# hailanyi/CPD

Hardware: AMD Instinct MI355X
Metric: frames/sec voxelize->sparse3D->BEV->NMS, 160k-pt Waymo cloud (higher is better)
Workload: dtype f32 (split-fp16 x2 on the fp16 MFMA pipe: 3 products, fp32 accumulate)

## Files before the change

### cpd_amd/_lib.py

```python
import ctypes
import os

import torch

_HERE = os.path.dirname(os.path.abspath(__file__))
LIB_PATH = os.environ.get("CPD_HIP_LIB", os.path.join(_HERE, "csrc", "libcpd_hip.so"))

CPD_ERRORS = {-1: "CPD_ERR_ARG", -2: "CPD_ERR_WORKSPACE", -3: "CPD_ERR_LAUNCH", -4: "CPD_ERR_UNSUPPORTED"}


class CpdHipError(RuntimeError):
    pass


_lib = None

_VP, _I, _F, _SZ = ctypes.c_void_p, ctypes.c_int, ctypes.c_float, ctypes.c_size_t
_D = ctypes.c_double
_I3 = ctypes.POINTER(ctypes.c_int32)
_FP = ctypes.POINTER(ctypes.c_float)

SIGNATURES = {
    "cpd_launch_log_enable": (None, [_I]),
    "cpd_launch_log_note": (None, [ctypes.c_char_p]),
# ... 34 lines not shown
    "cpd_conv3x3_rows_scaled": (_I, [_VP, _I, _I, _I, _I, _I, _VP, _I, _VP, _VP, _VP, _I, _I, _VP, _I, _I, _VP, _VP]),
    "cpd_conv3x3_rows_ranged": (_I, [_VP, _I, _I, _I, _I, _I, _VP, _I, _VP, _VP, _VP, _I, _I, _VP, _I, _I, _VP, _VP, _VP]),
    "cpd_gather_conv_ranged": (_I, [_VP, _I, _I, _I, _VP, _VP, _VP, _I, _I, _I, _VP, _VP, _VP, _I, _I, _VP, _I, _VP, _I, _I, _VP, _VP, _VP]),
    "cpd_gather_conv_ws": (_I, [_VP, _I, _I, _I, _VP, _VP, _VP, _I, _I, _I, _VP, _VP, _VP, _I, _I, _VP, _I, _VP, _I, _I, _VP, _VP, _VP, _SZ, _VP]),
    "cpd_gather_conv_split_bytes": (_SZ, [_I, _I, _I, _I, _I, _I]),
    "cpd_absmax_rows": (_I, [_VP, _I, ctypes.c_longlong, _I, _VP, _VP]),
    "cpd_densify_nchw": (_I, [_VP, _VP, _I, _I, _I, _I3, _VP, _VP]),
    "cpd_densify_nhwc": (_I, [_VP, _VP, _I, _I, _I, _I3, _VP, _VP]),
    "cpd_densify_nhwc_cd": (_I, [_VP, _VP, _I, _I, _I, _I3, _VP, _VP]),
    "cpd_densify_nhwc_rows": (_I, [_VP, _VP, _I, _I, _I, _I3, _VP, _VP]),
    "cpd_densify_nhwc_clear": (_I, [_VP, _I, _I, _I, _I3, _VP, _VP]),
    "cpd_rulebook_conv2d": (_I, [_I, _I, _I, _I, _I, _I, _I, _VP, _VP]),
    "cpd_center_decode_workspace_bytes": (_SZ, [_I, _I, _I, _I]),
    "cpd_center_decode": (_I, [_VP, _VP, _VP, _VP, _VP, _I, ctypes.c_longlong, _I, _I, _I, _I, _I, _I, _F, _FP, _FP, _FP, _F,
                               _VP, _VP, _VP, _VP, _VP, _SZ, _VP]),
    "cpd_boxes_overlap_bev": (_I, [_VP, _I, _VP, _I, _VP, _VP]),
    "cpd_boxes_iou_bev": (_I, [_VP, _I, _VP, _I, _VP, _VP]),
    "cpd_boxes_iou3d": (_I, [_VP, _I, _VP, _I, _VP, _VP]),
    "cpd_nms_workspace_bytes": (_SZ, [_I]),
    "cpd_nms_rotated": (_I, [_VP, _I, _F, _VP, _VP, _VP, _SZ, _VP]),
    "cpd_nms_normal": (_I, [_VP, _I, _F, _VP, _VP, _VP, _SZ, _VP]),
    "cpd_nms_batch": (_I, [_VP, _VP, _I, _I, _F, _I, _VP, _VP, _VP, _SZ, _VP]),
    "cpd_nms_batch_first": (_I, [_VP, _VP, _I, _I, _F, _I, _I, _I, _VP, _VP, _VP, _VP, _SZ, _VP]),
    "cpd_nms_batch_where": (_I, [_VP, _VP, _VP, _I, _I, _F, _I, _VP, _VP, _VP, _SZ, _VP]),
    "cpd_rank_scores": (_I, [_VP, _I, _VP, _VP, _I, _I, _F, _I, _I, _VP, _VP, _VP, _VP, _VP]),
    "cpd_select_boxes": (_I, [_VP, _VP, _VP, _VP, _VP, _I, _I, _I, _I, _VP, _VP, _VP, _VP, _VP]),
    "cpd_boxes_iou_bev_cpu": (_I, [_VP, _I, _VP, _I, _VP]),
    "cpd_col_reduce_workspace_bytes": (_SZ, [_I, _I]),
    "cpd_col_sum": (_I, [_VP, _I, _I, _I, _VP, _VP, _SZ, _VP]),
    "cpd_bn_stats": (_I, [_VP, _I, _I, _I, _VP, _VP, _VP, _SZ, _VP]),
# ... 126 lines not shown
```

### cpd_amd/csrc/decode.hip

```cpp
#include "common.h"

namespace {

struct MapView {
    const float *p;
    int pix, ch;
    __device__ __forceinline__ MapView sample(int b, long long sample_stride) const {
        return MapView{p + (size_t)b * sample_stride, pix, ch};
    }
    __device__ __forceinline__ float at(int pixel, int channel) const {
        return p[(size_t)pixel * pix + (size_t)channel * ch];
    }
};

__device__ __forceinline__ uint32_t f2key(float f) {
    uint32_t u = __float_as_uint(f);
    return (u & 0x80000000u) ? ~u : (u | 0x80000000u);
}
__device__ __forceinline__ float key2f(uint32_t k) {
    uint32_t u = (k & 0x80000000u) ? (k & 0x7fffffffu) : ~k;
    return __uint_as_float(u);
}
__device__ __forceinline__ float sigmoidf(float x) { return 1.0f / (1.0f + expf(-x)); }

// ... 144 lines not shown
__global__ void __launch_bounds__(1024) topk_class_kernel(MapView hm_all, long long sample_stride, int num_class, int hw,
                                                          int K, float *__restrict__ s1, int32_t *__restrict__ i1) {
    __shared__ TopkSmem sm;
    __shared__ TopkHist hist;
    const int cls = blockIdx.x, b = blockIdx.y;
    const MapView hm = hm_all.sample(b, sample_stride);
    if (!block_topk_logits(hm, cls, hw, K, hist, sm)) block_topk(hw, K, SigKey{hm, cls}, sm);
    const size_t o = ((size_t)b * num_class + cls) * K;
    for (int k = threadIdx.x; k < K; k += blockDim.x) {
        unsigned long long p = sm.packed[k];
        s1[o + k] = key2f((uint32_t)(p >> 32));
        i1[o + k] = (int32_t)(~(uint32_t)p);
    }
}

struct DecodeParams {
    MapView center, center_z, dim, rot;
    long long sample_stride;
    int num_class, h, w, K;
    float stride, vx, vy, lox, loy;
    float lim[6];
    float score_thresh;
};

__global__ void __launch_bounds__(1024) decode_kernel(DecodeParams q, const float *__restrict__ s1,
                                                      const int32_t *__restrict__ i1, float *__restrict__ boxes,
                                                      float *__restrict__ scores, int32_t *__restrict__ labels,
                                                      int32_t *__restrict__ n_out) {
    __shared__ TopkSmem sm;
    const int K = q.K;
    const int bsmp = blockIdx.x;
    s1 += (size_t)bsmp * q.num_class * K;
    i1 += (size_t)bsmp * q.num_class * K;
    boxes += (size_t)bsmp * K * 7;
    scores += (size_t)bsmp * K;
    labels += (size_t)bsmp * K;
    n_out += bsmp;
    q.center = q.center.sample(bsmp, q.sample_stride);
    q.center_z = q.center_z.sample(bsmp, q.sample_stride);
    q.dim = q.dim.sample(bsmp, q.sample_stride);
    q.rot = q.rot.sample(bsmp, q.sample_stride);
    {
        const int n = q.num_class * K;
        for (int i2 = threadIdx.x; i2 < n; i2 += blockDim.x) {
            const int c = i2 / K, j = i2 - c * K;
            const uint32_t key = f2key(s1[i2]);
            int rank = j;
            for (int c2 = 0; c2 < q.num_class; ++c2) {
                if (c2 == c) continue;
                const float *l = s1 + (size_t)c2 * K;
                int lo = 0, hi = K;
                while (lo < hi) {
                    const int mid = (lo + hi) >> 1;
                    const uint32_t km = f2key(l[mid]);
                    if (c2 < c ? km >= key : km > key) lo = mid + 1; else hi = mid;
                }
                rank += lo;
            }
            if (rank < K) sm.packed[rank] = ((unsigned long long)key << 32) | (uint32_t)(~(uint32_t)i2);
        }
        __syncthreads();
    }
    const int k = threadIdx.x;
    float bx[7];
    float sc = 0.f;
    int cls = 0;
    uint32_t keep = 0;
    if (k < K) {
        unsigned long long p = sm.packed[k];
        sc = key2f((uint32_t)(p >> 32));
        const int i2 = (int)(~(uint32_t)p);
        cls = i2 / K;
        const int ind = i1[i2];
        const float xs = (float)(ind % q.w), ys = (float)(ind / q.w);
        bx[0] = (xs + q.center.at(ind, 0)) * q.stride * q.vx + q.lox;
        bx[1] = (ys + q.center.at(ind, 1)) * q.stride * q.vy + q.loy;
        bx[2] = q.center_z.at(ind, 0);
        bx[3] = expf(q.dim.at(ind, 0));
        bx[4] = expf(q.dim.at(ind, 1));
        bx[5] = expf(q.dim.at(ind, 2));
        bx[6] = atan2f(q.rot.at(ind, 1), q.rot.at(ind, 0));
        bool ok = bx[0] >= q.lim[0] && bx[1] >= q.lim[1] && bx[2] >= q.lim[2] && bx[0] <= q.lim[3] &&
                  bx[1] <= q.lim[4] && bx[2] <= q.lim[5];
        ok = ok && (sc > q.score_thresh);
        keep = ok ? 1u : 0u;
    }
    __syncthreads();
    uint32_t tot;
    uint32_t pos = block_excl_scan(keep, sm.scan, &tot);
    if (keep) {
#pragma unroll
        for (int c = 0; c < 7; ++c) boxes[(size_t)pos * 7 + c] = bx[c];
        scores[pos] = sc;
        labels[pos] = cls;
    }
    if (threadIdx.x == 0) *n_out = (int32_t)tot;
}

}

extern "C" size_t cpd_center_decode_workspace_bytes(int batch, int num_class, int hw, int k) {
    if (batch <= 0 || num_class <= 0 || hw <= 0 || k <= 0) return 0;
    return cpd_align((size_t)batch * num_class * k * 4) * 2;
}

extern "C" int cpd_center_decode(const float *hm, const float *center, const float *center_z, const float *dim,
                                 const float *rot, int batch, long long sample_stride, int pix_stride, int ch_stride,
                                 int num_class, int h, int w, int k,
                                 float feature_map_stride, const float voxel_xy[2], const float range_lo_xy[2],
                                 const float limit_range[6], float score_thresh, float *boxes, float *scores,
                                 int32_t *labels, int32_t *n_out, void *workspace, size_t workspace_bytes,
                                 cpd_stream_t stream) {
    if (!hm || !center || !center_z || !dim || !rot || !boxes || !scores || !labels || !n_out || !workspace ||
// ... 2 lines not shown
    const long long hw = (long long)h * w;
    if (k > 1024 || k > hw || (long long)num_class * k > (1 << 24) || hw >= (1ll << 31)) return CPD_ERR_UNSUPPORTED;
    if (workspace_bytes < cpd_center_decode_workspace_bytes(batch, num_class, (int)hw, k)) return CPD_ERR_WORKSPACE;
    hipStream_t s = cpd_s(stream);
    float *s1 = (float *)workspace;
    int32_t *i1 = (int32_t *)((char *)workspace + cpd_align((size_t)batch * num_class * k * 4));
    topk_class_kernel<<<dim3(num_class, batch), 1024, 0, s>>>(MapView{hm, pix_stride, ch_stride}, sample_stride, num_class,
                                                              (int)hw, k, s1, i1);
    DecodeParams q;
    q.center = MapView{center, pix_stride, ch_stride};
    q.center_z = MapView{center_z, pix_stride, ch_stride};
    q.dim = MapView{dim, pix_stride, ch_stride};
    q.rot = MapView{rot, pix_stride, ch_stride};
    q.sample_stride = sample_stride;
    q.num_class = num_class; q.h = h; q.w = w; q.K = k;
    q.stride = feature_map_stride; q.vx = voxel_xy[0]; q.vy = voxel_xy[1];
    q.lox = range_lo_xy[0]; q.loy = range_lo_xy[1];
    for (int i = 0; i < 6; ++i) q.lim[i] = limit_range[i];
    q.score_thresh = score_thresh;
    decode_kernel<<<batch, 1024, 0, s>>>(q, s1, i1, boxes, scores, labels, n_out);
    return cpd_check_launch();
}
```

### cpd_amd/engine.py

```python
import contextlib
import math
from dataclasses import dataclass, field
from typing import Dict, List

import torch

from . import _lib, ops


@dataclass
class ModelConfig:
    point_cloud_range: List[float] = field(default_factory=lambda: [-75.2, -75.2, -2.0, 75.2, 75.2, 4.0])
    voxel_size: List[float] = field(default_factory=lambda: [0.1, 0.1, 0.15])
    max_points_per_voxel: int = 5
    max_voxels: int = 1000000
    num_point_features: int = 5
    num_filters: List[int] = field(default_factory=lambda: [16, 32, 64, 128])
    out_features: int = 128
    bev_layer_nums: List[int] = field(default_factory=lambda: [5, 5])
    bev_layer_strides: List[int] = field(default_factory=lambda: [1, 2])
    bev_num_filters: List[int] = field(default_factory=lambda: [128, 256])
    bev_upsample_strides: List[int] = field(default_factory=lambda: [1, 2])
    bev_num_upsample_filters: List[int] = field(default_factory=lambda: [256, 256])
    shared_conv_channel: int = 64
# ... 17 lines not shown
    voxelizer_group: int = 64
    batched_voxelizer_min_frames: int = 2
    row_order: str = "taps"
    row_order_brick: tuple = (8, 8)
    row_order_level0: bool = False
    chunked_rulebooks: bool = True
    plan_channels: tuple = (32, 64)
    plan_tile_rows: int = 256
    plan_rulebooks: bool = False
    row_order_chunk: int = 4096
    row_order_min_rows: int = 65536
    index_side_stream: bool = True
    deblock_side_stream: bool = True
    deblock_side_stream_max_frames: int = 8
    index_side_stream_max_frames: int = 1 << 30

    @property
    def grid_zyx(self):
        return ops.voxel_grid_size(self.voxel_size, self.point_cloud_range)

    @property
    def sparse_shape(self):
        g = self.grid_zyx
        return [g[0] + 1, g[1], g[2]]

    def head_names(self):
        return list(self.head_order) + ["hm"]

    def head_out(self, name):
        return self.num_class if name == "hm" else self.head_channels[name]
# ... 90 lines not shown
    if conv_bias is not None:
        shift = shift + conv_bias.double() * scale
    return scale.float(), shift.float()


class _Layer:
    __slots__ = ("w", "kv", "c_in", "c_out", "scale", "shift", "relu")

    def __init__(self, w_kio, scale, shift, relu, device):
        w_kio = w_kio.to(device=device, dtype=torch.float32).contiguous()
        self.kv, self.c_in, self.c_out = w_kio.shape
        self.w = ops.pack_weight(w_kio)
        self.scale = scale.to(device).contiguous() if scale is not None else None
        self.shift = shift.to(device).contiguous() if shift is not None else None
        self.relu = relu


class CenterPointEngine:

    SPARSE_BN_EPS = 1e-3
    BEV_BN_EPS = 1e-3
    HEAD_BN_EPS = 1e-5

    def __init__(self, cfg: ModelConfig, state_dict: Dict[str, torch.Tensor], device="cuda", host_results=False):
        self.cfg = cfg
        self.device = torch.device(device)
        self.host_results = bool(host_results)
        self.sd = state_dict
        self.voxelizer = ops.Voxelizer(cfg.voxel_size, cfg.point_cloud_range, cfg.num_point_features,
                                       cfg.max_points_per_voxel, cfg.max_voxels, device=self.device)
# ... 73 lines not shown
        for hi, name in enumerate(names):
            q = p + "heads_list.0.%s." % name
            w = sd[q + "0.0.weight"]
            w1.append(w.permute(2, 3, 1, 0).reshape(9, sc, sc))
            s, t = _fold_bn(sd, q + "0.1", self.HEAD_BN_EPS, sd.get(q + "0.0.bias"))
            s1.append(s); t1.append(t)
            wo = sd[q + "1.weight"]
            co = wo.shape[0]
            w2[:, hi * sc:(hi + 1) * sc, col:col + co] = wo.permute(2, 3, 1, 0).reshape(9, sc, co)
            b2[col:col + co] = sd[q + "1.bias"]
            self.head_slices[name] = (col, co)
            col += co
        self.head1 = _Layer(torch.cat(w1, dim=2), torch.cat(s1), torch.cat(t1), True, dev)
        self.head2 = _Layer(w2, None, b2, False, dev)
        self.head_ld = 16 * ((n_out + 15) // 16)

    def _final_shape(self):
        shape = self.cfg.sparse_shape
        for stage in ["conv2", "conv3", "conv4", "conv_out"]:
            k, s, pd = _DOWN[stage]
            shape = ops.conv_out_shape(shape, k, s, pd)
        return shape

    def _final_depth(self):
        return self._final_shape()[0]

    def _side_stream(self):
        return _lib.side_stream(self.device, "index")

    def _range_reset(self):
        self._rb = None
        self._rb_next = 0
        if self.cfg.conv_math == "f16x2" and self.cfg.range_guard:
            if getattr(self, "_rb_pool", None) is None:
                n = 21 + sum(k + 1 for k in self.cfg.bev_layer_nums) + 1 + 3 + 16
                self._rb_pool = ops.absmax_blocks(n, self.device)
            else:
                self._rb_pool.zero_()
        else:
            self._rb_pool = None

    def _range_new(self):
        if self._rb_pool is None:
            return None
        if self._rb_next >= self._rb_pool.shape[0]:
            raise RuntimeError("range guard: this model launches more convolutions per step than the %d absmax blocks the engine "
                               "sized from its config (engine._range_reset)" % self._rb_pool.shape[0])
        b = self._rb_pool[self._rb_next]
        self._rb_next += 1
        return b

    RANGE_STICKY_STEPS = 16

    def _range_exceeded_flag(self):
        if self._rb_pool is None:
            return None
        thr = 0x46800000 if getattr(self, "_rb_scaled", False) else 0x47000000
        return (self._rb_pool.max() >= thr).to(torch.int32).view(1)

    def _conv(self, layer, x, nbr, n_out, residual=None, out=None, out_row_map=None, out_col_group=0, dense=False, out_rb="new",
              in_pairs=False, out_pairs=False, res_pairs=False):
        rb_in = self._rb if getattr(self, "_rb_scaled", False) else None
        rb_out = self._range_new() if out_rb == "new" else out_rb
        y = ops.gather_conv(x, layer.c_in, layer.w, nbr, layer.kv, n_out, layer.c_out, layer.scale, layer.shift,
                            residual, layer.relu, out=out, out_row_map=out_row_map, out_col_group=out_col_group,
                            dense=dense, math=self.cfg.conv_math, in_absmax=rb_in, out_absmax=rb_out,
                            in_pairs=in_pairs, out_pairs=out_pairs, res_pairs=res_pairs)
        self._rb = rb_out
        return y

    def _blocks(self, blocks, x, nbr, pairs=False):
        n = x.shape[0]
        for c1, c2 in blocks:
            y = self._conv(c1, x, nbr, n, in_pairs=pairs, out_pairs=pairs)
            x = self._conv(c2, y, nbr, n, residual=x, in_pairs=pairs, out_pairs=pairs, res_pairs=pairs)
        return x

    def backbone3d(self, feats, coords, batch, index=None, pair_rows=False, export_levels=True, canonical0=False, dense_pairs=False):
        pairs = bool(pair_rows) and self.cfg.conv_math == "f16x2"
        want = (lambda name: name in export_levels) if isinstance(export_levels, (tuple, list, set)) else (lambda name: bool(export_levels))
        self.level_indexes = {}
        L = self.sparse
# ... 137 lines not shown
                ok = ok and convs[0].c_out % 128 == 0 and convs[0].c_in % 32 == 0
            for cv in (convs if stride == 1 else convs[1:]):
                ok = ok and ops.conv3x3_rows_tile(batch, cur_h, cur_w, cv.c_in, cv.c_out) in ((128, 128), (128, 64))
            ok = ok and de.c_out % 128 == 0 and c_up % 32 == 0
            widest = max(widest, max(cv.c_out for cv in convs))
        c_cat = sum(cfg.bev_num_upsample_filters)
        ok = ok and self._head_pairs_ok(batch, h, w, c_cat)
        widest = max(widest, c_cat, getattr(getattr(self, "head1", None), "c_out", 0))
        ok = ok and batch * h * w * widest * 4 + (w + 300) * widest * 4 < 0xfff00000
        self._bev_cache[key] = bool(ok)
        return bool(ok)

    def _head_pairs_ok(self, batch, h, w, c_cat):
        return (ops.conv3x3_rows_tile(batch, h, w, c_cat, self.shared.c_out) in ((256, 64), (128, 64)) and
                ops.conv3x3_rows_tile(batch, h, w, self.head1.c_in, self.head1.c_out) in ((256, 64), (128, 64)) and
                ops.conv3x3_rows_tile(batch, h, w, self.head2.c_in, self.head2.c_out) in ((256, 16), (128, 16)))

    def bev_and_head(self, dense_rows, batch, h, w, pairs=False):
        cfg = self.cfg
        pk = dict(in_pairs=True, out_pairs=True) if pairs else {}
        T = self._bev_tables(batch, h, w)
        if getattr(self, "_rb_stage", None) != "backbone":
            self._range_reset()
        self._rb_stage = None
        cat_rb = self._range_new()
        n_full = batch * h * w
        c_cat = sum(cfg.bev_num_upsample_filters)
        cat = torch.empty((n_full, c_cat), dtype=torch.float32, device=self.device)
        x = dense_rows
        col = 0
        cur_h, cur_w = h, w
        side = self._side_stream() if (cfg.index_side_stream and cfg.deblock_side_stream and dense_rows.is_cuda
                                       and batch <= cfg.deblock_side_stream_max_frames) else None
# ... 26 lines not shown
                if aside:
                    side.wait_event(ev)
                if u == 1:
                    self._conv(de, x, None, n_lvl, out=dst, dense=True, out_rb=cat_rb, **pk)
                elif u == 2 and (ho * 2, wo * 2) == (h, w):
                    self._conv(de, x, None, n_lvl, out=dst, out_row_map=T["up2"], out_col_group=c_up, dense=True, out_rb=cat_rb, **pk)
                else:
                    raise NotImplementedError("upsample stride outside the shipped configs")
                if aside:
                    joins.append(side.record_event())
            self._rb = x_rb
            col += c_up
        for ev in joins:
            main.wait_event(ev)
        self._rb = cat_rb
        return cat, self._head_rows(cat, batch, h, w, T, pairs)

    def _head_rows(self, cat, batch, h, w, T, pairs):
        pk = dict(in_pairs=True, out_pairs=True) if pairs else {}
        n_full = batch * h * w
        s = self._conv(self.shared, cat, T["s1"][0], n_full, dense=True, **pk)
        h1 = self._conv(self.head1, s, T["s1"][0], n_full, dense=True, **pk)
        out = torch.empty((n_full, self.head_ld), dtype=torch.float32, device=self.device)
        self._conv(self.head2, h1, T["s1"][0], n_full, out=out, dense=pairs, in_pairs=pairs)
        return out

    def decode_and_nms(self, head_rows, batch, h, w, raw=False):
        cfg = self.cfg
        ld = self.head_ld
        sl = self.head_slices
        base = head_rows
        boxes, scores, labels, counts = ops.center_decode(
            base[:, sl["hm"][0]:], base[:, sl["center"][0]:], base[:, sl["center_z"][0]:], base[:, sl["dim"][0]:],
            base[:, sl["rot"][0]:], ld, 1, cfg.num_class, h, w, cfg.max_obj_per_sample, float(cfg.feature_map_stride),
            cfg.voxel_size[:2], cfg.point_cloud_range[:2], cfg.post_center_limit_range, cfg.score_thresh, sync=False,
            batch=batch, sample_stride=h * w * ld)
        assert cfg.max_obj_per_sample <= cfg.nms_pre_maxsize
        keep, num_keep = ops.nms_batch(boxes, counts, cfg.nms_thresh)
        flag = self._range_exceeded_flag()
        ob, os_, ol, on, blk = ops.select_boxes(boxes, scores, labels, keep, num_keep, cfg.nms_post_maxsize, label_offset=1,
                                                packed=True, extra_ints=1)
        lay = blk._cpd_layout
        hdr = blk[:4 * lay["n_hdr"]].view(torch.int32)
        if flag is not None:
            hdr[batch:batch + 1].copy_(flag)
        whole = self.host_results and not raw
        host = blk.cpu() if whole else None
        ns = (ops.unpack_boxes(host, lay)[0] if whole else hdr).tolist()
        high = bool(ns[batch]) if flag is not None else False
        if getattr(self, "_rb_scaled", False):
            self._range_exceeded, self._range_high = False, high
# ... 68 lines not shown
            levels, (x, out_idx, out_shape) = self.backbone3d(feats, coords, batch, index=index0, canonical0=canonical0,
                                                              export_levels=proposals if proposals is not None else return_intermediates,
                                                              pair_rows=self.cfg.pair_rows and not self._rb_scaled, dense_pairs=dp)
            d, h, w = out_shape
            dp = dp and self.encoded_pairs
            dmap = None
            if self.cfg.persistent_dense_map and not return_intermediates:
                key = ("dense_map", d, h, w, x.shape[1])
                dmap = self._bev_cache.get(key)
                if dmap is None or dmap.batch < batch:
                    dmap = self._bev_cache[key] = ops.DenseMap(batch, out_shape, x.shape[1], self.device)
                dense = dmap.scatter(x, out_idx, batch).view(batch * h * w, d * x.shape[1])
            else:
                dense = ops.densify_nhwc(x, out_idx, batch, out_shape).view(batch * h * w, d * x.shape[1])
            self._dense_map = dmap
            cat, head = self.bev_and_head(dense, batch, h, w, pairs=dp)
            results = self.decode_and_nms(head, batch, h, w, raw=proposals is not None)
            if results is not None:
                break
            if self.range_reruns == 0:
                import warnings
                warnings.warn("cpd_amd: an activation reached 2^15 -- step re-run with the range-guarded f16x2 kernels; the engine "
                              "stays guarded for the next %d steps" % self.RANGE_STICKY_STEPS)
            self._rb_scaled = True
            self.range_reruns += 1
            self._guard_left = self.RANGE_STICKY_STEPS + 1
        if self._rb_scaled:
            self.range_guarded_steps += 1
            self._guard_left = self.RANGE_STICKY_STEPS if self._range_high else self._guard_left - 1
        self._rb_scaled = False
        if proposals is not None:
# ... 11 lines not shown
```

### cpd_amd/ops.py

```python
import ctypes

import torch

from . import _lib
from ._lib import check, farr, iarr, lib, ptr, stream


def _dev(t):
    return t.device


def _need_cuda(t, name):
    if not t.is_cuda:
        raise _lib.CpdHipError("%s must be a device (HIP) tensor" % name)


def voxel_grid_size(vsize_xyz, range_xyz):
    g = (ctypes.c_int32 * 3)()
    check(lib().cpd_voxel_grid_size(farr(vsize_xyz), farr(range_xyz), g), "cpd_voxel_grid_size")
    return [g[0], g[1], g[2]]


class Voxelizer:

# ... 245 lines not shown
    check(lib().cpd_pack_weight(ptr(w_kio), kv, cin, cout, ptr(packed), stream()), "cpd_pack_weight")
    return packed


CONV_MATH = {"f32": 0, "bf16x3": 2, "f16x2": 4}


def _gc_flags(dense, bf16x3, math):
    if math is not None:
        return (1 if dense else 0) | CONV_MATH[math]
    return (1 if dense else 0) | (2 if bf16x3 else 0)


def gather_conv(inp, c_in, packed_w, nbr, kv, n_out, c_out, scale=None, shift=None, residual=None, relu=False,
                out=None, out_row_map=None, out_col_group=0, dense=False, bf16x3=False, math=None, in_absmax=None, out_absmax=None,
                guard=False, in_pairs=False, out_pairs=False, res_pairs=False):
    _need_cuda(inp, "inp")
    assert inp.dim() == 2 and inp.stride(1) == 1
    if guard and in_absmax is None and (math == "f16x2") and c_in % 32 == 0:
        in_absmax = absmax_rows(inp, c_in)
    if out is None:
        out = torch.empty((n_out, c_out), dtype=torch.float32, device=inp.device)
    assert out.dim() == 2 and out.stride(1) == 1
    res_ld = 0
    if residual is not None:
        assert residual.dim() == 2 and residual.stride(1) == 1
        res_ld = residual.stride(0)
    flags = _gc_flags(dense, bf16x3, math) | (16 if in_pairs else 0) | (32 if out_pairs else 0) | (64 if res_pairs else 0)
    image = getattr(nbr, "image", None)
    if image is not None and (dense or not (flags & 0x70)) and out_row_map is None and kv == 9 and n_out == image[0] * image[1] * image[2] and inp.shape[0] == n_out:
        rc = lib().cpd_conv3x3_rows_ranged(
# ... 1 lines not shown
            ptr(scale), ptr(shift), ctypes.c_void_p(residual.data_ptr()) if residual is not None else None, res_ld,
            int(bool(relu)), ctypes.c_void_p(out.data_ptr()), out.stride(0), flags, ptr(in_absmax), ptr(out_absmax), stream())
        if rc != -4:
            check(rc, "cpd_conv3x3_rows")
            return out
    plan = getattr(nbr, "plan", None)
    if plan is not None and in_absmax is None and out_row_map is None and not out_col_group and lib().cpd_gather_conv_planned_supported(
            int(inp.shape[0]), int(n_out), int(c_in), int(c_out), int(inp.stride(0)), int(kv), flags):
        check(lib().cpd_gather_conv_planned(
            ctypes.c_void_p(inp.data_ptr()), inp.stride(0), inp.shape[0], c_in, ptr(packed_w), ptr(getattr(nbr, "tapmask", None)),
            ptr(plan[0]), ptr(plan[1]), ptr(plan[2]), plan[3], kv, n_out, c_out, ptr(scale), ptr(shift),
            ctypes.c_void_p(residual.data_ptr()) if residual is not None else None, res_ld, int(bool(relu)),
            ctypes.c_void_p(out.data_ptr()), out.stride(0), flags, ptr(out_absmax), stream()), "cpd_gather_conv_planned")
        return out
    ws, ws_bytes = None, 0
    if (flags & 6) and c_in % 32 == 0 and not out_col_group:
        ws_bytes = int(lib().cpd_gather_conv_split_bytes(int(n_out), int(c_in), int(c_out), int(inp.stride(0)), int(kv), flags))
        if ws_bytes:
            ws = torch.empty((ws_bytes // 4,), dtype=torch.float32, device=inp.device)
    check(lib().cpd_gather_conv_ws(
        ctypes.c_void_p(inp.data_ptr()), inp.stride(0), inp.shape[0], c_in, ptr(packed_w),
        ptr(nbr), ptr(getattr(nbr, "tapmask", None)), kv, n_out, c_out, ptr(scale), ptr(shift),
        ctypes.c_void_p(residual.data_ptr()) if residual is not None else None, res_ld, int(bool(relu)),
        ctypes.c_void_p(out.data_ptr()), out.stride(0), ptr(out_row_map), int(out_col_group), flags,
        ptr(in_absmax), ptr(out_absmax), ptr(ws), ws_bytes, stream()),
        "cpd_gather_conv")
    return out


def rows_to_pairs(x):
    n, c = x.shape
# ... 184 lines not shown
    boxes = torch.empty((batch, k, 7), dtype=torch.float32, device=dev)
    scores = torch.empty((batch, k), dtype=torch.float32, device=dev)
    labels = torch.empty((batch, k), dtype=torch.int32, device=dev)
    n_out = torch.zeros((batch,), dtype=torch.int32, device=dev)
    ws = torch.empty(lib().cpd_center_decode_workspace_bytes(batch, num_class, h * w, k), dtype=torch.uint8, device=dev)
    check(lib().cpd_center_decode(
        ctypes.c_void_p(hm.data_ptr()), ctypes.c_void_p(center.data_ptr()), ctypes.c_void_p(center_z.data_ptr()),
        ctypes.c_void_p(dim.data_ptr()), ctypes.c_void_p(rot.data_ptr()), int(batch), int(sample_stride), pix_stride,
        ch_stride, num_class, h, w, k, float(feature_map_stride), farr(voxel_xy), farr(range_lo_xy), farr(limit_range),
        float(score_thresh), ptr(boxes), ptr(scores), ptr(labels), ptr(n_out), ptr(ws), ws.numel(), stream()),
        "cpd_center_decode")
    if not sync or batch != 1:
        return boxes, scores, labels, n_out
    n = int(n_out.item())
    return boxes[0, :n], scores[0, :n], labels[0, :n], n


def nms_batch(boxes, counts, thresh, normal=False):
    boxes = boxes.contiguous()
    batch, cap = boxes.shape[0], boxes.shape[1]
    keep = torch.empty((batch, cap), dtype=torch.int64, device=boxes.device)
    num = torch.zeros((batch,), dtype=torch.int32, device=boxes.device)
    ws = torch.empty(batch * lib().cpd_nms_workspace_bytes(cap), dtype=torch.uint8, device=boxes.device)
    check(lib().cpd_nms_batch(ptr(boxes), ptr(counts), batch, cap, float(thresh), 1 if normal else 0, ptr(keep), ptr(num),
                              ptr(ws), ws.numel(), stream()), "cpd_nms_batch")
    return keep, num


def nms_batch_first(boxes, counts, thresh, max_keep, row_limit, normal=False):
    boxes = boxes.contiguous()
# ... 161 lines not shown
```

### include/cpd_hip.h

```cpp
#ifndef CPD_HIP_H
#define CPD_HIP_H

#include <stddef.h>
#include <stdint.h>

#ifdef __cplusplus
extern "C" {
#endif

typedef void *cpd_stream_t;

#define CPD_OK 0
#define CPD_ERR_ARG (-1)
#define CPD_ERR_WORKSPACE (-2)
#define CPD_ERR_LAUNCH (-3)
#define CPD_ERR_UNSUPPORTED (-4)

const char *cpd_version(void);
void cpd_launch_log_enable(int on);
void cpd_launch_log_note(const char *kernel);
size_t cpd_launch_log_dump(char *buf, size_t cap);
int cpd_last_hip_error(void);

int cpd_voxel_grid_size(const float vsize_xyz[3], const float range_xyz[6], int32_t grid_zyx[3]);
// ... 100 lines not shown
                           cpd_stream_t stream);
int cpd_densify_nhwc_cd(const float *feat, const int32_t *indices, int n, int c, int batch,
                        const int32_t shape_zyx[3], float *out, cpd_stream_t stream);
int cpd_rulebook_conv2d(int batch, int h, int w, int kh, int kw, int stride, int pad,
                        int32_t *nbr, cpd_stream_t stream);

size_t cpd_center_decode_workspace_bytes(int batch, int num_class, int hw, int k);
int cpd_center_decode(const float *hm, const float *center, const float *center_z,
                      const float *dim, const float *rot, int batch, long long sample_stride,
                      int pix_stride, int ch_stride, int num_class, int h, int w, int k,
                      float feature_map_stride,
                      const float voxel_xy[2], const float range_lo_xy[2],
                      const float limit_range[6], float score_thresh, float *boxes, float *scores,
                      int32_t *labels, int32_t *n_out, void *workspace, size_t workspace_bytes,
                      cpd_stream_t stream);

int cpd_boxes_overlap_bev(const float *a, int n, const float *b, int m, float *out,
                          cpd_stream_t stream);
int cpd_boxes_iou_bev(const float *a, int n, const float *b, int m, float *out,
                      cpd_stream_t stream);
int cpd_boxes_iou3d(const float *a, int n, const float *b, int m, float *out,
                    cpd_stream_t stream);
size_t cpd_nms_workspace_bytes(int n);
int cpd_nms_rotated(const float *boxes, int n, float thresh, int64_t *keep, int32_t *num_keep,
                    void *workspace, size_t workspace_bytes, cpd_stream_t stream);
int cpd_nms_normal(const float *boxes, int n, float thresh, int64_t *keep, int32_t *num_keep,
                   void *workspace, size_t workspace_bytes, cpd_stream_t stream);
int cpd_nms_batch(const float *boxes, const int32_t *counts, int batch, int capacity, float thresh,
                  int normal, int64_t *keep, int32_t *num_keep, void *workspace,
                  size_t workspace_bytes, cpd_stream_t stream);
// ... 231 lines not shown
```

Before: 1230.

## Compute regression head only at top-K heatmap winners via sparse gather conv

```diff
diff --git a/cpd_amd/_lib.py b/cpd_amd/_lib.py
--- a/cpd_amd/_lib.py
+++ b/cpd_amd/_lib.py
@@ -72,6 +72,8 @@
     "cpd_center_decode_workspace_bytes": (_SZ, [_I, _I, _I, _I]),
     "cpd_center_decode": (_I, [_VP, _VP, _VP, _VP, _VP, _I, ctypes.c_longlong, _I, _I, _I, _I, _I, _I, _F, _FP, _FP, _FP, _F,
                                _VP, _VP, _VP, _VP, _VP, _SZ, _VP]),
+    "cpd_center_topk": (_I, [_VP, _I, ctypes.c_longlong, _I, _I, _I, _I, _I, _I, _VP, _VP, _VP, _VP, _VP, _VP, _SZ, _VP]),
+    "cpd_center_decode_rows": (_I, [_VP, _I, _I3, _VP, _VP, _VP, _I, _I, _I, _F, _FP, _FP, _FP, _F, _VP, _VP, _VP, _VP, _VP]),
     "cpd_boxes_overlap_bev": (_I, [_VP, _I, _VP, _I, _VP, _VP]),
     "cpd_boxes_iou_bev": (_I, [_VP, _I, _VP, _I, _VP, _VP]),
     "cpd_boxes_iou3d": (_I, [_VP, _I, _VP, _I, _VP, _VP]),
diff --git a/cpd_amd/csrc/decode.hip b/cpd_amd/csrc/decode.hip
--- a/cpd_amd/csrc/decode.hip
+++ b/cpd_amd/csrc/decode.hip
@@ -182,14 +182,67 @@
     }
 }
 
+struct DecodeGeom {
+    int w;
+    float stride, vx, vy, lox, loy;
+    float lim[6];
+    float score_thresh;
+};
 struct DecodeParams {
     MapView center, center_z, dim, rot;
     long long sample_stride;
     int num_class, h, w, K;
-    float stride, vx, vy, lox, loy;
-    float lim[6];
-    float score_thresh;
-};
+    DecodeGeom g;
+};
+
+__device__ __forceinline__ bool decode_box(const DecodeGeom &g, int ind, float sc, const float reg[8], float bx[7]) {
+    const float xs = (float)(ind % g.w), ys = (float)(ind / g.w);
+    bx[0] = (xs + reg[0]) * g.stride * g.vx + g.lox;
+    bx[1] = (ys + reg[1]) * g.stride * g.vy + g.loy;
+    bx[2] = reg[2];
+    bx[3] = expf(reg[3]);
+    bx[4] = expf(reg[4]);
+    bx[5] = expf(reg[5]);
+    bx[6] = atan2f(reg[7], reg[6]);
+    bool ok = bx[0] >= g.lim[0] && bx[1] >= g.lim[1] && bx[2] >= g.lim[2] && bx[0] <= g.lim[3] &&
+              bx[1] <= g.lim[4] && bx[2] <= g.lim[5];
+    return ok && (sc > g.score_thresh);
+}
+
+__device__ __forceinline__ void compact_boxes(uint32_t keep, const float bx[7], float sc, int cls, uint32_t *scan, float *__restrict__ boxes,
+                                              float *__restrict__ scores, int32_t *__restrict__ labels, int32_t *__restrict__ n_out) {
+    uint32_t tot;
+    uint32_t pos = block_excl_scan(keep, scan, &tot);
+    if (keep) {
+#pragma unroll
+        for (int c = 0; c < 7; ++c) boxes[(size_t)pos * 7 + c] = bx[c];
+        scores[pos] = sc;
+        labels[pos] = cls;
+    }
+    if (threadIdx.x == 0) *n_out = (int32_t)tot;
+}
+
+__device__ __forceinline__ void merge_ranks(int num_class, int K, const float *__restrict__ s1, TopkSmem &sm) {
+    const int n = num_class * K;
+    for (int i2 = threadIdx.x; i2 < n; i2 += blockDim.x) {
+        const int c = i2 / K, j = i2 - c * K;
+        const uint32_t key = f2key(s1[i2]);
+        int rank = j;
+        for (int c2 = 0; c2 < num_class; ++c2) {
+            if (c2 == c) continue;
+            const float *l = s1 + (size_t)c2 * K;
+            int lo = 0, hi = K;
+            while (lo < hi) {
+                const int mid = (lo + hi) >> 1;
+                const uint32_t km = f2key(l[mid]);
+                if (c2 < c ? km >= key : km > key) lo = mid + 1; else hi = mid;
+            }
+            rank += lo;
+        }
+        if (rank < K) sm.packed[rank] = ((unsigned long long)key << 32) | (uint32_t)(~(uint32_t)i2);
+    }
+    __syncthreads();
+}
 
 __global__ void __launch_bounds__(1024) decode_kernel(DecodeParams q, const float *__restrict__ s1,
                                                       const int32_t *__restrict__ i1, float *__restrict__ boxes,
@@ -208,27 +261,7 @@
     q.center_z = q.center_z.sample(bsmp, q.sample_stride);
     q.dim = q.dim.sample(bsmp, q.sample_stride);
     q.rot = q.rot.sample(bsmp, q.sample_stride);
-    {
-        const int n = q.num_class * K;
-        for (int i2 = threadIdx.x; i2 < n; i2 += blockDim.x) {
-            const int c = i2 / K, j = i2 - c * K;
-            const uint32_t key = f2key(s1[i2]);
-            int rank = j;
-            for (int c2 = 0; c2 < q.num_class; ++c2) {
-                if (c2 == c) continue;
-                const float *l = s1 + (size_t)c2 * K;
-                int lo = 0, hi = K;
-                while (lo < hi) {
-                    const int mid = (lo + hi) >> 1;
-                    const uint32_t km = f2key(l[mid]);
-                    if (c2 < c ? km >= key : km > key) lo = mid + 1; else hi = mid;
-                }
-                rank += lo;
-            }
-            if (rank < K) sm.packed[rank] = ((unsigned long long)key << 32) | (uint32_t)(~(uint32_t)i2);
-        }
-        __syncthreads();
-    }
+    merge_ranks(q.num_class, K, s1, sm);
     const int k = threadIdx.x;
     float bx[7];
     float sc = 0.f;
@@ -240,31 +273,86 @@
         const int i2 = (int)(~(uint32_t)p);
         cls = i2 / K;
         const int ind = i1[i2];
-        const float xs = (float)(ind % q.w), ys = (float)(ind / q.w);
-        bx[0] = (xs + q.center.at(ind, 0)) * q.stride * q.vx + q.lox;
-        bx[1] = (ys + q.center.at(ind, 1)) * q.stride * q.vy + q.loy;
-        bx[2] = q.center_z.at(ind, 0);
-        bx[3] = expf(q.dim.at(ind, 0));
-        bx[4] = expf(q.dim.at(ind, 1));
-        bx[5] = expf(q.dim.at(ind, 2));
-        bx[6] = atan2f(q.rot.at(ind, 1), q.rot.at(ind, 0));
-        bool ok = bx[0] >= q.lim[0] && bx[1] >= q.lim[1] && bx[2] >= q.lim[2] && bx[0] <= q.lim[3] &&
-                  bx[1] <= q.lim[4] && bx[2] <= q.lim[5];
-        ok = ok && (sc > q.score_thresh);
-        keep = ok ? 1u : 0u;
-    }
-    __syncthreads();
-    uint32_t tot;
-    uint32_t pos = block_excl_scan(keep, sm.scan, &tot);
-    if (keep) {
-#pragma unroll
-        for (int c = 0; c < 7; ++c) boxes[(size_t)pos * 7 + c] = bx[c];
-        scores[pos] = sc;
-        labels[pos] = cls;
-    }
-    if (threadIdx.x == 0) *n_out = (int32_t)tot;
-}
-
+        const float reg[8] = {q.center.at(ind, 0), q.center.at(ind, 1), q.center_z.at(ind, 0), q.dim.at(ind, 0),
+                              q.dim.at(ind, 1), q.dim.at(ind, 2), q.rot.at(ind, 0), q.rot.at(ind, 1)};
+        keep = decode_box(q.g, ind, sc, reg, bx) ? 1u : 0u;
+    }
+    __syncthreads();
+    compact_boxes(keep, bx, sc, cls, sm.scan, boxes, scores, labels, n_out);
+}
+
+__global__ void __launch_bounds__(1024) merge_tables_kernel(int num_class, int h, int w, int K, int batch, const float *__restrict__ s1,
+                                                            const int32_t *__restrict__ i1, float *__restrict__ win_scores,
+                                                            int32_t *__restrict__ win_labels, int32_t *__restrict__ win_pixels,
+                                                            int32_t *__restrict__ nbr_hidden, int32_t *__restrict__ nbr_out) {
+    __shared__ TopkSmem sm;
+    __shared__ int32_t pix[1024];
+    const int bsmp = blockIdx.x;
+    s1 += (size_t)bsmp * num_class * K;
+    i1 += (size_t)bsmp * num_class * K;
+    merge_ranks(num_class, K, s1, sm);
+    const int k = threadIdx.x;
+    if (k < K) {
+        const unsigned long long p = sm.packed[k];
+        const int i2 = (int)(~(uint32_t)p);
+        const int ind = i1[i2];
+        pix[k] = ind;
+        win_scores[(size_t)bsmp * K + k] = key2f((uint32_t)(p >> 32));
+        win_labels[(size_t)bsmp * K + k] = i2 / K;
+        win_pixels[(size_t)bsmp * K + k] = ind;
+    }
+    __syncthreads();
+    const size_t n_hid = (size_t)batch * K * 9, n_win = (size_t)batch * K;
+    const int32_t hid0 = (int32_t)((size_t)bsmp * K * 9), map0 = (int32_t)((size_t)bsmp * h * w);
+    for (int e = threadIdx.x; e < K * 81; e += blockDim.x) {
+        const int j = e / 81, r = e - j * 81;
+        const int tp = r / 9, t = r - tp * 9;
+        const int ind = pix[j];
+        const int y = ind / w + t / 3 - 1, x = ind % w + t % 3 - 1;
+        const bool in = (unsigned)y < (unsigned)h && (unsigned)x < (unsigned)w;
+        const int yy = y + tp / 3 - 1, xx = x + tp % 3 - 1;
+        int32_t v = -1;
+        if (in && (unsigned)yy < (unsigned)h && (unsigned)xx < (unsigned)w) v = map0 + yy * w + xx;
+        nbr_hidden[(size_t)tp * n_hid + hid0 + j * 9 + t] = v;
+        if (tp == 0) nbr_out[(size_t)t * n_win + (size_t)bsmp * K + j] = in ? hid0 + j * 9 + t : -1;
+    }
+}
+
+__global__ void __launch_bounds__(1024) decode_rows_kernel(DecodeGeom g, int K, const float *__restrict__ rows, int ld, int c_center,
+                                                           int c_z, int c_dim, int c_rot, const float *__restrict__ win_scores,
+                                                           const int32_t *__restrict__ win_labels, const int32_t *__restrict__ win_pixels,
+                                                           float *__restrict__ boxes, float *__restrict__ scores,
+                                                           int32_t *__restrict__ labels, int32_t *__restrict__ n_out) {
+    __shared__ uint32_t scan[17];
+    const int bsmp = blockIdx.x;
+    const size_t o = (size_t)bsmp * K;
+    const int k = threadIdx.x;
+    float bx[7];
+    float sc = 0.f;
+    int cls = 0;
+    uint32_t keep = 0;
+    if (k < K) {
+        sc = win_scores[o + k];
+        cls = win_labels[o + k];
+        const float *r = rows + (o + k) * (size_t)ld;
+        const float reg[8] = {r[c_center], r[c_center + 1], r[c_z], r[c_dim], r[c_dim + 1], r[c_dim + 2], r[c_rot], r[c_rot + 1]};
+        keep = decode_box(g, win_pixels[o + k], sc, reg, bx) ? 1u : 0u;
+    }
+    __syncthreads();
+    compact_boxes(keep, bx, sc, cls, scan, boxes + o * 7, scores + o, labels + o, n_out + bsmp);
+}
+
+}
+
+static DecodeGeom decode_geom(int w, float feature_map_stride, const float voxel_xy[2], const float range_lo_xy[2],
+                              const float limit_range[6], float score_thresh) {
+    DecodeGeom g;
+    g.w = w;
+    g.stride = feature_map_stride; g.vx = voxel_xy[0]; g.vy = voxel_xy[1];
+    g.lox = range_lo_xy[0]; g.loy = range_lo_xy[1];
+    for (int i = 0; i < 6; ++i) g.lim[i] = limit_range[i];
+    g.score_thresh = score_thresh;
+    return g;
 }
 
 extern "C" size_t cpd_center_decode_workspace_bytes(int batch, int num_class, int hw, int k) {
@@ -297,10 +385,44 @@
     q.rot = MapView{rot, pix_stride, ch_stride};
     q.sample_stride = sample_stride;
     q.num_class = num_class; q.h = h; q.w = w; q.K = k;
-    q.stride = feature_map_stride; q.vx = voxel_xy[0]; q.vy = voxel_xy[1];
-    q.lox = range_lo_xy[0]; q.loy = range_lo_xy[1];
-    for (int i = 0; i < 6; ++i) q.lim[i] = limit_range[i];
-    q.score_thresh = score_thresh;
+    q.g = decode_geom(w, feature_map_stride, voxel_xy, range_lo_xy, limit_range, score_thresh);
     decode_kernel<<<batch, 1024, 0, s>>>(q, s1, i1, boxes, scores, labels, n_out);
     return cpd_check_launch();
 }
+
+extern "C" int cpd_center_topk(const float *hm, int batch, long long sample_stride, int pix_stride, int ch_stride, int num_class, int h,
+                               int w, int k, float *win_scores, int32_t *win_labels, int32_t *win_pixels, int32_t *nbr_hidden,
+                               int32_t *nbr_out, void *workspace, size_t workspace_bytes, cpd_stream_t stream) {
+    if (!hm || !win_scores || !win_labels || !win_pixels || !nbr_hidden || !nbr_out || !workspace || batch <= 0 || num_class <= 0 ||
+        h <= 0 || w <= 0 || k <= 0)
+        return CPD_ERR_ARG;
+    const long long hw = (long long)h * w;
+    if (k > 1024 || k > hw || (long long)num_class * k > (1 << 24) || (long long)batch * hw >= (1ll << 31) ||
+        (long long)batch * k * 9 >= (1ll << 31))
+        return CPD_ERR_UNSUPPORTED;
+    if (workspace_bytes < cpd_center_decode_workspace_bytes(batch, num_class, (int)hw, k)) return CPD_ERR_WORKSPACE;
+    hipStream_t s = cpd_s(stream);
+    float *s1 = (float *)workspace;
+    int32_t *i1 = (int32_t *)((char *)workspace + cpd_align((size_t)batch * num_class * k * 4));
+    topk_class_kernel<<<dim3(num_class, batch), 1024, 0, s>>>(MapView{hm, pix_stride, ch_stride}, sample_stride, num_class,
+                                                              (int)hw, k, s1, i1);
+    merge_tables_kernel<<<batch, 1024, 0, s>>>(num_class, h, w, k, batch, s1, i1, win_scores, win_labels, win_pixels, nbr_hidden, nbr_out);
+    return cpd_check_launch();
+}
+
+extern "C" int cpd_center_decode_rows(const float *rows, int ld, const int32_t cols[4], const float *win_scores,
+                                      const int32_t *win_labels, const int32_t *win_pixels, int batch, int w, int k,
+                                      float feature_map_stride, const float voxel_xy[2], const float range_lo_xy[2],
+                                      const float limit_range[6], float score_thresh, float *boxes, float *scores, int32_t *labels,
+                                      int32_t *n_out, cpd_stream_t stream) {
+    if (!rows || !cols || !win_scores || !win_labels || !win_pixels || !boxes || !scores || !labels || !n_out || !voxel_xy ||
+        !range_lo_xy || !limit_range || batch <= 0 || w <= 0 || k <= 0 || ld <= 0)
+        return CPD_ERR_ARG;
+    if (cols[0] < 0 || cols[0] + 2 > ld || cols[1] < 0 || cols[1] + 1 > ld || cols[2] < 0 || cols[2] + 3 > ld || cols[3] < 0 || cols[3] + 2 > ld)
+        return CPD_ERR_ARG;
+    if (k > 1024) return CPD_ERR_UNSUPPORTED;
+    decode_rows_kernel<<<batch, 1024, 0, cpd_s(stream)>>>(decode_geom(w, feature_map_stride, voxel_xy, range_lo_xy, limit_range, score_thresh),
+                                                          k, rows, ld, cols[0], cols[1], cols[2], cols[3], win_scores, win_labels,
+                                                          win_pixels, boxes, scores, labels, n_out);
+    return cpd_check_launch();
+}
diff --git a/cpd_amd/engine.py b/cpd_amd/engine.py
--- a/cpd_amd/engine.py
+++ b/cpd_amd/engine.py
@@ -55,6 +55,8 @@
     deblock_side_stream: bool = True
     deblock_side_stream_max_frames: int = 8
     index_side_stream_max_frames: int = 1 << 30
+    sparse_head: bool = True
+    sparse_head_min_frames: int = 4
 
     @property
     def grid_zyx(self):
@@ -175,6 +177,13 @@
         self.scale = scale.to(device).contiguous() if scale is not None else None
         self.shift = shift.to(device).contiguous() if shift is not None else None
         self.relu = relu
+
+
+class SparseHeadRows:
+    __slots__ = ("reg", "scores", "labels", "pixels")
+
+    def __init__(self, reg, scores, labels, pixels):
+        self.reg, self.scores, self.labels, self.pixels = reg, scores, labels, pixels
 
 
 class CenterPointEngine:
@@ -278,6 +287,27 @@
         self.head1 = _Layer(torch.cat(w1, dim=2), torch.cat(s1), torch.cat(t1), True, dev)
         self.head2 = _Layer(w2, None, b2, False, dev)
         self.head_ld = 16 * ((n_out + 15) // 16)
+        self._head_parts = (names, sc, w1, s1, t1, w2, b2)
+
+    def _sparse_head_layers(self):
+        if getattr(self, "head1_reg", None) is None:
+            names, sc, w1, s1, t1, w2, b2 = self._head_parts
+            dev = self.device
+            if names[-1] != "hm":
+                raise NotImplementedError("sparse head tail: the heat-map branch is expected last (ModelConfig.head_names)")
+            nr = len(names) - 1
+            c0, co = self.head_slices["hm"]
+            self.head1_hm = _Layer(w1[-1], s1[-1], t1[-1], True, dev)
+            self.head2_hm = _Layer(w2[:, nr * sc:, c0:c0 + co].contiguous(), None, b2[c0:c0 + co], False, dev)
+            self.hm_ld = 16 * ((co + 15) // 16)
+            self.reg_ld = 32 * ((c0 + 31) // 32)
+            w2r = torch.zeros(9, nr * sc, self.reg_ld)
+            w2r[:, :, :c0] = w2[:, :nr * sc, :c0]
+            b2r = torch.zeros(self.reg_ld)
+            b2r[:c0] = b2[:c0]
+            self.head1_reg = _Layer(torch.cat(w1[:-1], dim=2), torch.cat(s1[:-1]), torch.cat(t1[:-1]), True, dev)
+            self.head2_reg = _Layer(w2r, None, b2r, False, dev)
+        return self.head1_hm, self.head2_hm, self.head1_reg, self.head2_reg
 
     def _final_shape(self):
         shape = self.cfg.sparse_shape
@@ -297,7 +327,7 @@
         self._rb_next = 0
         if self.cfg.conv_math == "f16x2" and self.cfg.range_guard:
             if getattr(self, "_rb_pool", None) is None:
-                n = 21 + sum(k + 1 for k in self.cfg.bev_layer_nums) + 1 + 3 + 16
+                n = 21 + sum(k + 1 for k in self.cfg.bev_layer_nums) + 1 + 5 + 16
                 self._rb_pool = ops.absmax_blocks(n, self.device)
             else:
                 self._rb_pool.zero_()
@@ -323,13 +353,13 @@
         return (self._rb_pool.max() >= thr).to(torch.int32).view(1)
 
     def _conv(self, layer, x, nbr, n_out, residual=None, out=None, out_row_map=None, out_col_group=0, dense=False, out_rb="new",
-              in_pairs=False, out_pairs=False, res_pairs=False):
+              in_pairs=False, out_pairs=False, res_pairs=False, tap_split=True):
         rb_in = self._rb if getattr(self, "_rb_scaled", False) else None
         rb_out = self._range_new() if out_rb == "new" else out_rb
         y = ops.gather_conv(x, layer.c_in, layer.w, nbr, layer.kv, n_out, layer.c_out, layer.scale, layer.shift,
                             residual, layer.relu, out=out, out_row_map=out_row_map, out_col_group=out_col_group,
                             dense=dense, math=self.cfg.conv_math, in_absmax=rb_in, out_absmax=rb_out,
-                            in_pairs=in_pairs, out_pairs=out_pairs, res_pairs=res_pairs)
+                            in_pairs=in_pairs, out_pairs=out_pairs, res_pairs=res_pairs, tap_split=tap_split)
         self._rb = rb_out
         return y
 
@@ -497,9 +527,11 @@
     def _head_pairs_ok(self, batch, h, w, c_cat):
         return (ops.conv3x3_rows_tile(batch, h, w, c_cat, self.shared.c_out) in ((256, 64), (128, 64)) and
                 ops.conv3x3_rows_tile(batch, h, w, self.head1.c_in, self.head1.c_out) in ((256, 64), (128, 64)) and
-                ops.conv3x3_rows_tile(batch, h, w, self.head2.c_in, self.head2.c_out) in ((256, 16), (128, 16)))
-
-    def bev_and_head(self, dense_rows, batch, h, w, pairs=False):
+                ops.conv3x3_rows_tile(batch, h, w, self.head2.c_in, self.head2.c_out) in ((256, 16), (128, 16)) and
+                ops.conv3x3_rows_tile(batch, h, w, self.head1.c_in, self.head1.c_in) in ((256, 64), (128, 64)) and
+                ops.conv3x3_rows_tile(batch, h, w, self.head1.c_in, self.cfg.num_class) in ((256, 16), (128, 16)))
+
+    def bev_and_head(self, dense_rows, batch, h, w, pairs=False, sparse_head=False):
         cfg = self.cfg
         pk = dict(in_pairs=True, out_pairs=True) if pairs else {}
         T = self._bev_tables(batch, h, w)
@@ -556,7 +588,7 @@
         for ev in joins:
             main.wait_event(ev)
         self._rb = cat_rb
-        return cat, self._head_rows(cat, batch, h, w, T, pairs)
+        return cat, (self._head_rows_sparse if sparse_head else self._head_rows)(cat, batch, h, w, T, pairs)
 
     def _head_rows(self, cat, batch, h, w, T, pairs):
         pk = dict(in_pairs=True, out_pairs=True) if pairs else {}
@@ -567,16 +599,45 @@
         self._conv(self.head2, h1, T["s1"][0], n_full, out=out, dense=pairs, in_pairs=pairs)
         return out
 
+    def sparse_head_ok(self, batch, return_intermediates=False):
+        cfg = self.cfg
+        return (cfg.sparse_head and not return_intermediates and batch >= cfg.sparse_head_min_frames and
+                type(self)._head_rows is CenterPointEngine._head_rows and type(self).decode_and_nms is CenterPointEngine.decode_and_nms)
+
+    def _head_rows_sparse(self, cat, batch, h, w, T, pairs):
+        cfg = self.cfg
+        pk = dict(in_pairs=True, out_pairs=True) if pairs else {}
+        n_full = batch * h * w
+        K = cfg.max_obj_per_sample
+        head1_hm, head2_hm, head1_reg, head2_reg = self._sparse_head_layers()
+        s = self._conv(self.shared, cat, T["s1"][0], n_full, dense=True, **pk)
+        s_rb = self._rb
+        hh = self._conv(head1_hm, s, T["s1"][0], n_full, dense=True, **pk)
+        hm = torch.empty((n_full, self.hm_ld), dtype=torch.float32, device=self.device)
+        self._conv(head2_hm, hh, T["s1"][0], n_full, out=hm, dense=pairs, in_pairs=pairs)
+        scores, labels, pixels, nbr_hidden, nbr_out = ops.center_topk(hm, self.hm_ld, 1, cfg.num_class, h, w, K, batch=batch,
+                                                                      sample_stride=h * w * self.hm_ld)
+        self._rb = s_rb
+        hid = self._conv(head1_reg, s, nbr_hidden, batch * K * 9, tap_split=False, **pk)
+        reg = self._conv(head2_reg, hid, nbr_out, batch * K, in_pairs=pairs, tap_split=False)
+        return SparseHeadRows(reg, scores, labels, pixels)
+
     def decode_and_nms(self, head_rows, batch, h, w, raw=False):
         cfg = self.cfg
         ld = self.head_ld
         sl = self.head_slices
         base = head_rows
-        boxes, scores, labels, counts = ops.center_decode(
-            base[:, sl["hm"][0]:], base[:, sl["center"][0]:], base[:, sl["center_z"][0]:], base[:, sl["dim"][0]:],
-            base[:, sl["rot"][0]:], ld, 1, cfg.num_class, h, w, cfg.max_obj_per_sample, float(cfg.feature_map_stride),
-            cfg.voxel_size[:2], cfg.point_cloud_range[:2], cfg.post_center_limit_range, cfg.score_thresh, sync=False,
-            batch=batch, sample_stride=h * w * ld)
+        if isinstance(head_rows, SparseHeadRows):
+            boxes, scores, labels, counts = ops.center_decode_rows(
+                head_rows.reg, [sl["center"][0], sl["center_z"][0], sl["dim"][0], sl["rot"][0]], head_rows.scores, head_rows.labels,
+                head_rows.pixels, w, float(cfg.feature_map_stride), cfg.voxel_size[:2], cfg.point_cloud_range[:2],
+                cfg.post_center_limit_range, cfg.score_thresh)
+        else:
+            boxes, scores, labels, counts = ops.center_decode(
+                base[:, sl["hm"][0]:], base[:, sl["center"][0]:], base[:, sl["center_z"][0]:], base[:, sl["dim"][0]:],
+                base[:, sl["rot"][0]:], ld, 1, cfg.num_class, h, w, cfg.max_obj_per_sample, float(cfg.feature_map_stride),
+                cfg.voxel_size[:2], cfg.point_cloud_range[:2], cfg.post_center_limit_range, cfg.score_thresh, sync=False,
+                batch=batch, sample_stride=h * w * ld)
         assert cfg.max_obj_per_sample <= cfg.nms_pre_maxsize
         keep, num_keep = ops.nms_batch(boxes, counts, cfg.nms_thresh)
         flag = self._range_exceeded_flag()
@@ -675,7 +736,10 @@
             else:
                 dense = ops.densify_nhwc(x, out_idx, batch, out_shape).view(batch * h * w, d * x.shape[1])
             self._dense_map = dmap
-            cat, head = self.bev_and_head(dense, batch, h, w, pairs=dp)
+            if self.sparse_head_ok(batch, return_intermediates):
+                cat, head = self.bev_and_head(dense, batch, h, w, pairs=dp, sparse_head=True)
+            else:
+                cat, head = self.bev_and_head(dense, batch, h, w, pairs=dp)
             results = self.decode_and_nms(head, batch, h, w, raw=proposals is not None)
             if results is not None:
                 break
diff --git a/cpd_amd/ops.py b/cpd_amd/ops.py
--- a/cpd_amd/ops.py
+++ b/cpd_amd/ops.py
@@ -283,7 +283,7 @@
 
 def gather_conv(inp, c_in, packed_w, nbr, kv, n_out, c_out, scale=None, shift=None, residual=None, relu=False,
                 out=None, out_row_map=None, out_col_group=0, dense=False, bf16x3=False, math=None, in_absmax=None, out_absmax=None,
-                guard=False, in_pairs=False, out_pairs=False, res_pairs=False):
+                guard=False, in_pairs=False, out_pairs=False, res_pairs=False, tap_split=True):
     _need_cuda(inp, "inp")
     assert inp.dim() == 2 and inp.stride(1) == 1
     if guard and in_absmax is None and (math == "f16x2") and c_in % 32 == 0:
@@ -315,7 +315,7 @@
             ctypes.c_void_p(out.data_ptr()), out.stride(0), flags, ptr(out_absmax), stream()), "cpd_gather_conv_planned")
         return out
     ws, ws_bytes = None, 0
-    if (flags & 6) and c_in % 32 == 0 and not out_col_group:
+    if tap_split and (flags & 6) and c_in % 32 == 0 and not out_col_group:
         ws_bytes = int(lib().cpd_gather_conv_split_bytes(int(n_out), int(c_in), int(c_out), int(inp.stride(0)), int(kv), flags))
         if ws_bytes:
             ws = torch.empty((ws_bytes // 4,), dtype=torch.float32, device=inp.device)
@@ -530,6 +530,37 @@
         return boxes, scores, labels, n_out
     n = int(n_out.item())
     return boxes[0, :n], scores[0, :n], labels[0, :n], n
+
+
+def center_topk(hm, pix_stride, ch_stride, num_class, h, w, k, batch=1, sample_stride=0):
+    dev = hm.device
+    scores = torch.empty((batch, k), dtype=torch.float32, device=dev)
+    labels = torch.empty((batch, k), dtype=torch.int32, device=dev)
+    pixels = torch.empty((batch, k), dtype=torch.int32, device=dev)
+    nbr_hidden = torch.empty((9, batch * k * 9), dtype=torch.int32, device=dev)
+    nbr_out = torch.empty((9, batch * k), dtype=torch.int32, device=dev)
+    ws = torch.empty(lib().cpd_center_decode_workspace_bytes(batch, num_class, h * w, k), dtype=torch.uint8, device=dev)
+    check(lib().cpd_center_topk(ctypes.c_void_p(hm.data_ptr()), int(batch), int(sample_stride), pix_stride, ch_stride, num_class, h, w, k,
+                                ptr(scores), ptr(labels), ptr(pixels), ptr(nbr_hidden), ptr(nbr_out), ptr(ws), ws.numel(), stream()),
+          "cpd_center_topk")
+    return scores, labels, pixels, nbr_hidden, nbr_out
+
+
+def center_decode_rows(rows, cols, win_scores, win_labels, win_pixels, w, feature_map_stride, voxel_xy, range_lo_xy, limit_range,
+                       score_thresh):
+    assert rows.dim() == 2 and rows.stride(1) == 1 and rows.dtype == torch.float32
+    batch, k = win_scores.shape
+    assert rows.shape[0] == batch * k
+    dev = rows.device
+    boxes = torch.empty((batch, k, 7), dtype=torch.float32, device=dev)
+    scores = torch.empty((batch, k), dtype=torch.float32, device=dev)
+    labels = torch.empty((batch, k), dtype=torch.int32, device=dev)
+    n_out = torch.zeros((batch,), dtype=torch.int32, device=dev)
+    check(lib().cpd_center_decode_rows(
+        ctypes.c_void_p(rows.data_ptr()), rows.stride(0), iarr(cols), ptr(win_scores), ptr(win_labels), ptr(win_pixels), int(batch), int(w),
+        int(k), float(feature_map_stride), farr(voxel_xy), farr(range_lo_xy), farr(limit_range), float(score_thresh), ptr(boxes),
+        ptr(scores), ptr(labels), ptr(n_out), stream()), "cpd_center_decode_rows")
+    return boxes, scores, labels, n_out
 
 
 def nms_batch(boxes, counts, thresh, normal=False):
diff --git a/include/cpd_hip.h b/include/cpd_hip.h
--- a/include/cpd_hip.h
+++ b/include/cpd_hip.h
@@ -138,6 +138,16 @@
                       const float limit_range[6], float score_thresh, float *boxes, float *scores,
                       int32_t *labels, int32_t *n_out, void *workspace, size_t workspace_bytes,
                       cpd_stream_t stream);
+int cpd_center_topk(const float *hm, int batch, long long sample_stride, int pix_stride, int ch_stride,
+                    int num_class, int h, int w, int k, float *win_scores, int32_t *win_labels,
+                    int32_t *win_pixels, int32_t *nbr_hidden, int32_t *nbr_out, void *workspace,
+                    size_t workspace_bytes, cpd_stream_t stream);
+int cpd_center_decode_rows(const float *rows, int ld, const int32_t cols[4], const float *win_scores,
+                           const int32_t *win_labels, const int32_t *win_pixels, int batch, int w, int k,
+                           float feature_map_stride, const float voxel_xy[2],
+                           const float range_lo_xy[2], const float limit_range[6], float score_thresh,
+                           float *boxes, float *scores, int32_t *labels, int32_t *n_out,
+                           cpd_stream_t stream);
 
 int cpd_boxes_overlap_bev(const float *a, int n, const float *b, int m, float *out,
                           cpd_stream_t stream);
```

After: 1271, median of 6. +3.3%, better.
